# sebastianffx/stainlib

Hardware: AMD Instinct MI355X
Metric: 1024x1024 H&E tiles/sec normalized (Macenko) (higher is better)
Workload: dtype f32; 1 GPU; configs[1]: batch of 512 tiles 1024x1024x3 uint8 per GPU, Macenko transform (fit once outside the timed region), tiles resident in HBM; tiles_per_gpu=512, failed_tiles=0

## Files before the change

stainlib_amd/csrc/stats_finish.hpp:

```cpp
#pragma once
#include "stats_selection.hpp"
#include "stats_sweeps.hpp"

namespace sl {

struct SampleAngleKey {
    const uint32_t* sample; TabView tab; float V[6]; int cps_log2; int P; float ylimf;
    __device__ __forceinline__ float operator()(int b) const {
        if (sample_absent(b, cps_log2, P)) return nan_f();
        return of_word(sample[b]);
    }
    __device__ __forceinline__ float of_word(uint32_t s) const {
        const uint32_t r = s & 255u, g = (s >> 8) & 255u, bl = (s >> 16) & 255u;
        const bool tissue = is_tissue_f(tab.gam(r), tab.gam(g), tab.gam(bl), ylimf);
        const float k = angle_key(V, tab.odf(r), tab.odf(g), tab.odf(bl));
        return tissue ? k : nan_f();
    }
    __device__ __forceinline__ bool present(int b, int n_sample) const { return b < n_sample && !sample_absent(b, cps_log2, P); }
};
struct SampleConcKey {
    const uint32_t* sample; TabView tab; LassoK L; int cps_log2; int P; int col;
    __device__ __forceinline__ void both(int b, float& c1, float& c2) const {
        if (sample_absent(b, cps_log2, P)) { c1 = c2 = nan_f(); return; }
        of_word(sample[b], c1, c2);
    }
    __device__ __forceinline__ void of_word(uint32_t s, float& c1, float& c2) const {
        lasso2(L, tab.odf(s & 255u), tab.odf((s >> 8) & 255u), tab.odf((s >> 16) & 255u), c1, c2);
    }
    __device__ __forceinline__ bool present(int b, int n_sample) const { return b < n_sample && !sample_absent(b, cps_log2, P); }
    __device__ __forceinline__ float operator()(int b) const {
        float c1, c2;
        both(b, c1, c2);
        return col == 0 ? c1 : c2;
    }
};
struct AngleTileKey {
    const uint8_t* src; TabView tab; float V[6]; float ylimf;
    __device__ __forceinline__ float operator()(int p) const {
        const uint32_t r = src[3 * (size_t)p], g = src[3 * (size_t)p + 1], b = src[3 * (size_t)p + 2];
        if (!is_tissue_f(tab.gam(r), tab.gam(g), tab.gam(b), ylimf)) return nan_f();
        return angle_key(V, tab.odf(r), tab.odf(g), tab.odf(b));
    }
};
struct ConcTileKey {
    const uint8_t* src; TabView tab; LassoK L; int col;
    __device__ __forceinline__ float operator()(int p) const {
        float c1, c2;
        lasso2(L, tab.odf(src[3 * (size_t)p]), tab.odf(src[3 * (size_t)p + 1]), tab.odf(src[3 * (size_t)p + 2]), c1, c2);
        return col == 0 ? c1 : c2;
    }
};
struct RawConcKey2 {
    const uint32_t* raw; TabView tab; LassoK L;
    __device__ __forceinline__ void operator()(int i, float& k0, float& k1) const {
        const uint32_t s = raw[i];
        lasso2(L, tab.odf(s & 255u), tab.odf((s >> 8) & 255u), tab.odf((s >> 16) & 255u), k0, k1);
    }
};

struct CandKey {
    const float* cand;
    __device__ __forceinline__ float operator()(int i) const { return cand[i]; }
};

template <class Key2>
__device__ __forceinline__ void wg_refine(int n_raw, const Key2& key2, const float* lo, const float* hi, float* cand0,
                                          float* cand1, uint32_t cap_list, uint32_t* n_lt , uint32_t* n_in ,
                                          SelScratch& S, uint32_t* n_valid = nullptr ) {
    if (threadIdx.x < 4) S.misc[12 + threadIdx.x] = 0;
    if (threadIdx.x == 4) S.misc[8] = 0;
    __syncthreads();
    const int lane = threadIdx.x & 63;
    uint32_t lt0 = 0, lt1 = 0, nv = 0;
    constexpr int U = 4;
    const int step = (int)blockDim.x * U;
    for (int i0 = (int)(threadIdx.x - lane) * U; i0 < n_raw; i0 += step) {
        float k0[U], k1[U];
        unsigned long long m0[U], m1[U];
        uint32_t tot0 = 0, tot1 = 0;
#pragma unroll
        for (int u = 0; u < U; ++u) {
            const int i = i0 + u * 64 + lane;
            k0[u] = k1[u] = nan_f();
            if (i < n_raw) key2(i, k0[u], k1[u]);
        }
// ... 233 lines not shown
        if (__builtin_expect(n + cnt > stage_cap, 0)) flush(lane);
        const uint32_t rank = __builtin_amdgcn_mbcnt_hi((uint32_t)(m >> 32), __builtin_amdgcn_mbcnt_lo((uint32_t)m, 0u));
#if defined(__HIP_DEVICE_COMPILE__)
        uint32_t sbase;
        asm("s_lshl2_add_u32 %0, %1, %2" : "=s"(sbase) : "s"(n), "s"(buf) : "scc");
        const uint32_t addr = sbase + 4u * rank;
        unsigned long long saved;
        asm volatile("s_mov_b64 %0, exec\n\ts_mov_b64 exec, %1\n\tds_write_b32 %2, %3\n\ts_mov_b64 exec, %0"
                     : "=&s"(saved) : "s"(m), "v"(addr), "v"(value) : "memory");
#else
        (void)rank; (void)value;
#endif
        n += cnt;
    }
};


constexpr uint32_t kFinTabBytes = 2048;
__device__ __forceinline__ uint32_t fin_stage_bytes(int nthreads) { return (uint32_t)((sizeof(RowTab) - kFinTabBytes) / (size_t)(nthreads / 64)); }

struct FinTab {
    uint32_t base;
    __device__ __forceinline__ uint32_t addr(uint32_t w, int k) const { return k == 0 ? ((w << 3) & 0x7f8u) : ((w >> (8 * k - 3)) & 0x7f8u); }
#if defined(__HIP_DEVICE_COMPILE__)
    __device__ __forceinline__ float2 gam_odf(uint32_t a) const {
        const v2f v = *(SL_LDS const v2f*)(base + a);
        return make_float2(v.x, v.y);
    }
    __device__ __forceinline__ float odf(uint32_t a) const { return *(SL_LDS const float*)(base + a + 4u); }
#else
    float2 gam_odf(uint32_t) const { return float2{}; }
    float odf(uint32_t) const { return 0.0f; }
#endif
    __device__ __forceinline__ TabView view() const { return TabView{base, 8u, 4u, 0u}; }
};
__device__ __forceinline__ void fin_tab_build(RowTab& tab) {
    float2* p = reinterpret_cast<float2*>(tab.e);
    float2 e = make_float2(0.0f, 0.0f);
    if (threadIdx.x < 256) e = p[threadIdx.x * 32];
    __syncthreads();
    if (threadIdx.x < 256) p[threadIdx.x] = e;
    __syncthreads();
}

template <int NT>
__device__ __forceinline__ void fin_tab_expand(RowTab& tab) {
    float2* p = reinterpret_cast<float2*>(tab.e);
    constexpr int PER = 256 * 32 / NT;
    float2 e[PER];
#pragma unroll
    for (int j = 0; j < PER; ++j) e[j] = p[threadIdx.x / 32 + j * (NT / 32)];
    __syncthreads();
#pragma unroll
    for (int j = 0; j < PER; ++j) p[threadIdx.x + j * NT] = e[j];
    __syncthreads();
}

struct WordAngleKey {
    FinTab T; float V[6]; float ylimf;
    __device__ __forceinline__ void of_word(uint32_t s, float& k0, float& k1, bool& valid) const {
        const float2 er = T.gam_odf(T.addr(s, 0)), eg = T.gam_odf(T.addr(s, 1)), eb = T.gam_odf(T.addr(s, 2));
        valid = is_tissue_f(er.x, eg.x, eb.x, ylimf);
        k0 = k1 = angle_key(V, er.y, eg.y, eb.y);
    }
};
struct WordConcKey {
    FinTab T; LassoK L;
    __device__ __forceinline__ void of_word(uint32_t s, float& k0, float& k1, bool& valid) const {
        lasso2(L, T.odf(T.addr(s, 0)), T.odf(T.addr(s, 1)), T.odf(T.addr(s, 2)), k0, k1);
        valid = true;
    }
};

__device__ __forceinline__ void lds_count_masked(unsigned long long m, uint32_t addr, uint32_t one) {
#if defined(__HIP_DEVICE_COMPILE__)
    unsigned long long saved;
    asm volatile("s_mov_b64 %0, exec\n\ts_mov_b64 exec, %1\n\tds_add_u32 %2, %3\n\ts_mov_b64 exec, %0"
                 : "=&s"(saved) : "s"(m), "v"(addr), "v"(one) : "memory");
#else
    (void)m; (void)addr; (void)one;
#endif
}

struct RefineOut { uint32_t n_lt[2], n_in[2], n_valid; PickScale ps; };
template <class WordKey2>
__device__ __forceinline__ RefineOut wg_refine_s(const uint32_t* raw, int n_raw, const WordKey2& key2, float lo0, float hi0, float lo1, float hi1,
                                                 float* cand0, float* cand1, uint32_t cap_list, uint32_t stage_lds, uint32_t stage_entries,
                                                 SelScratch& S) {
    const int tid = threadIdx.x, lane = tid & 63;
    if (tid < 5) S.misc[8 + tid] = 0;
    for (int i = tid; i < 1024; i += blockDim.x) S.hist[i] = 0;
    RefineOut r;
    r.ps.lo[0] = lo0; r.ps.lo[1] = lo1;
    r.ps.sc[0] = (hi0 > lo0 && lo0 > -INFINITY && hi0 < INFINITY) ? 512.0f * 0.999999f / (hi0 - lo0) : 0.0f;
    r.ps.sc[1] = (hi1 > lo1 && lo1 > -INFINITY && hi1 < INFINITY) ? 512.0f * 0.999999f / (hi1 - lo1) : 0.0f;
    __syncthreads();
    stage_lds = (uint32_t)__builtin_amdgcn_readfirstlane((int)stage_lds);
    RawSink s0{stage_lds, 0u, reinterpret_cast<uint32_t*>(cand0), &S.misc[11], nullptr, cap_list, stage_entries};
    RawSink s1{stage_lds + 4u * stage_entries, 0u, reinterpret_cast<uint32_t*>(cand1), &S.misc[12], nullptr, cap_list, stage_entries};
    const float vlo0 = in_vgpr(lo0), vhi0 = in_vgpr(hi0), vlo1 = in_vgpr(lo1), vhi1 = in_vgpr(hi1);
    const float psl0 = in_vgpr(r.ps.lo[0]), psc0 = in_vgpr(r.ps.sc[0]), psl1 = in_vgpr(r.ps.lo[1]), psc1 = in_vgpr(r.ps.sc[1]);
    const uint32_t hist_lds = lds_address(S.hist);
    uint32_t one = 1u;
    asm("" : "+v"(one));
    uint32_t lt0 = 0, lt1 = 0, nv = 0;
    constexpr int U = 4;
    const int step = (int)blockDim.x * U;
    const int last = n_raw > 0 ? n_raw - 1 : 0;
    int i0 = (tid - lane) * U;
    uint32_t wn[U];
#pragma unroll
    for (int u = 0; u < U; ++u) wn[u] = as_global(raw)[min(i0 + u * 64 + lane, last)];
    for (; i0 < n_raw; i0 += step) {
        uint32_t w[U];
#pragma unroll
        for (int u = 0; u < U; ++u) {
            w[u] = wn[u];
            wn[u] = as_global(raw)[min(i0 + step + u * 64 + lane, last)];
        }
#pragma unroll
        for (int u = 0; u < U; ++u) {
            float k0, k1;
            bool valid;
            key2.of_word(w[u], k0, k1, valid);
            const bool inb = i0 + u * 64 + lane < n_raw;
            const unsigned long long mv = __builtin_amdgcn_ballot_w64(valid) & __builtin_amdgcn_ballot_w64(inb);
            const unsigned long long l0 = __builtin_amdgcn_ballot_w64(k0 < vlo0) & mv, l1 = __builtin_amdgcn_ballot_w64(k1 < vlo1) & mv;
            const unsigned long long m0 = __builtin_amdgcn_ballot_w64(k0 <= vhi0) & ~l0 & mv, m1 = __builtin_amdgcn_ballot_w64(k1 <= vhi1) & ~l1 & mv;
            nv += (uint32_t)__popcll(mv);
            lt0 += (uint32_t)__popcll(l0);
            lt1 += (uint32_t)__popcll(l1);
            lds_count_masked(m0, hist_lds + 4u * (uint32_t)pick_bin(k0, psl0, psc0), one);
            lds_count_masked(m1, hist_lds + 2048u + 4u * (uint32_t)pick_bin(k1, psl1, psc1), one);
            s0.put_value(m0, __float_as_uint(k0), lane);
            s1.put_value(m1, __float_as_uint(k1), lane);
        }
    }
    s0.flush(lane);
    s1.flush(lane);
    if (lane == 0) { if (nv) atomicAdd(&S.misc[8], nv); if (lt0) atomicAdd(&S.misc[9], lt0); if (lt1) atomicAdd(&S.misc[10], lt1); }
    __threadfence_block();
    __syncthreads();
    r.n_lt[0] = S.misc[9]; r.n_lt[1] = S.misc[10]; r.n_in[0] = S.misc[11]; r.n_in[1] = S.misc[12]; r.n_valid = S.misc[8];
    __syncthreads();
    return r;
}

constexpr float kBoxZ = 3.6f;
template <int THREADS>
__device__ __forceinline__ void angle_brackets(const SampleAngleKey& key, int n_sample, double pct, float* lo, float* hi,
                                               SelScratch& S, float* box = nullptr, float zs = 1.0f) {
    constexpr int KPT = kMaxSample / THREADS;
    uint32_t ord[1][KPT];
#ifdef SL_DEBUG_SUBCLK
    long long bclk_t_ = wall_clock64();
#endif
    static_assert(KPT % kBrkBatch == 0, "");
#pragma unroll
    for (int j0 = 0; j0 < KPT; j0 += kBrkBatch) {
        uint32_t w[kBrkBatch];
#pragma unroll
        for (int g = 0; g < kBrkBatch; ++g) {
            const int b = (j0 + g) * THREADS + (int)threadIdx.x;
            w[g] = b < n_sample ? as_global(key.sample)[b] : 0u;
        }
#pragma unroll
        for (int g = 0; g < kBrkBatch; ++g) {
            const int b = (j0 + g) * THREADS + (int)threadIdx.x;
            const float k = key.of_word(w[g]);
            ord[0][j0 + g] = (k == k && key.present(b, n_sample)) ? f2ord(k) : kAbsent;
        }
    }
    SL_BCLK(5);
    const int set_of[2] = {0, 0};
    const double p2[2] = {100.0 - pct, pct};
    wg_brackets_regs<1, KPT, 2>(ord, set_of, p2, lo, hi, S, kBracketZ * zs);
    if (box) {
        const bool closed = (lo[0] > -INFINITY) & (hi[0] < INFINITY) & (lo[1] > -INFINITY) & (hi[1] < INFINITY);
        if (closed) {
#pragma unroll
            for (int b = 0; b < 2; ++b) {
                const float m = 0.5f * (lo[b] + hi[b]), r = (float)kBoxFrac * 0.5f * (hi[b] - lo[b]);
                box[2 * b] = m - r; box[2 * b + 1] = m + r;
            }
        } else {
            const double n = (double)S.misc[6], q = p2[0] / 100.0;
            const bool inside = n > 0.0 && floor(q * (n - 1.0) - (double)(kBoxZ * zs) * sqrt(fmax(q * (1.0 - q) * n, 0.0))) - 1.0 >= 0.0;
            float blo[2] = {-INFINITY, -INFINITY}, bhi[2] = {INFINITY, INFINITY};
            __syncthreads();
            if (inside) wg_brackets_regs<1, KPT, 2>(ord, set_of, p2, blo, bhi, S, kBoxZ * zs);
            box[0] = blo[0]; box[1] = bhi[0]; box[2] = blo[1]; box[3] = bhi[1];
        }
    }
}
template <int THREADS>
__device__ __forceinline__ void conc_brackets(const SampleConcKey& key, int n_sample, float* lo, float* hi, SelScratch& S, float zs = 1.0f) {
    constexpr int KPT = kMaxSample / THREADS;
    uint32_t ord[2][KPT];
#ifdef SL_DEBUG_SUBCLK
    long long bclk_t_ = wall_clock64();
#endif
    static_assert(KPT % kBrkBatch == 0, "");
#pragma unroll
    for (int j0 = 0; j0 < KPT; j0 += kBrkBatch) {
        uint32_t w[kBrkBatch];
#pragma unroll
        for (int g = 0; g < kBrkBatch; ++g) {
            const int b = (j0 + g) * THREADS + (int)threadIdx.x;
            w[g] = b < n_sample ? as_global(key.sample)[b] : 0u;
        }
#pragma unroll
        for (int g = 0; g < kBrkBatch; ++g) {
            const int b = (j0 + g) * THREADS + (int)threadIdx.x;
            float c1, c2;
            key.of_word(w[g], c1, c2);
            const bool have = key.present(b, n_sample);
            ord[0][j0 + g] = (have && c1 == c1) ? f2ord(c1) : kAbsent;
            ord[1][j0 + g] = (have && c2 == c2) ? f2ord(c2) : kAbsent;
        }
    }
    SL_BCLK(6);
    const int set_of[2] = {0, 1};
    const double p2[2] = {99.0, 99.0};
    wg_brackets_regs<2, KPT, 2>(ord, set_of, p2, lo, hi, S, kBracketZ * zs);
}

}
```

stainlib_amd/csrc/stats_fused.hpp:

```cpp
#pragma once
#include "stats_phase_kernels.hpp"
#include "stats_cube.hpp"
#include "stats_twosweep.hpp"

namespace sl {

struct FusedArgs {
    const uint8_t* rgb;
    uint8_t* out;
    int n_tiles;
    int P;
    int stride_log2;
    int n_sample;
    float ylimf;
    double lam;
    double pct;
    const double* M_tgt;
    const double* maxC_tgt;
    int cap_raw, cap_list;
    uint32_t* raw;
    int cap_ang;
    uint32_t* raw_ang;
    float* cand;
    uint32_t* sample;
// ... 273 lines not shown
    const int P = __builtin_amdgcn_readfirstlane(P_), stream = __builtin_amdgcn_readfirstlane(stream_);
    const double lam = uni_d(lam_);
    const int tid = threadIdx.x;
    const TabReaderB TB = TabReaderB::make_at(FusedLds<NT>::tab);
    const int nch = (P + 3) >> 2;
    ApplyK K;
    apply_consts(sh.M, sh.maxC, M_tgt, maxC_tgt, lam, K);
    int t, c0, c1;
    fused_geometry<NT>(nch, tid, t, c0, c1);
    if (c0 >= c1) return;
    if (K.fast) {
        if (stream) apply_sweep<ALIGNED, true, TabReaderB, true>(src, dst, P, c0, c1, t, kFusedThreads, TB, K);
        else apply_sweep<ALIGNED, true, TabReaderB, false>(src, dst, P, c0, c1, t, kFusedThreads, TB, K);
    } else {
        if (stream) apply_sweep<ALIGNED, false, TabReaderB, true>(src, dst, P, c0, c1, t, kFusedThreads, TB, K);
        else apply_sweep<ALIGNED, false, TabReaderB, false>(src, dst, P, c0, c1, t, kFusedThreads, TB, K);
    }
}

template <int NT, bool ALIGNED>
__device__ __noinline__ void fused_sweep2_cube(FusedShared<NT>* shp, const uint8_t* src_, uint32_t* rawl_, uint32_t* rawa_, int P_, int cap_raw_, int cap_ang_,
                                               float ylimf_, int stream_) {
    FusedShared<NT>& sh = *shp;
    const uint8_t* src = uni_ptr(src_);
    uint32_t* rawl = uni_ptr(rawl_);
    uint32_t* rawa = uni_ptr(rawa_);
    const int P = __builtin_amdgcn_readfirstlane(P_), cap_raw = __builtin_amdgcn_readfirstlane(cap_raw_), stream = __builtin_amdgcn_readfirstlane(stream_);
    const int cap_ang = __builtin_amdgcn_readfirstlane(cap_ang_);
    const float ylimf = uni(ylimf_);
    const int tid = threadIdx.x, wave = tid >> 6;
    const TabReaderB TB = TabReaderB::make_at(FusedLds<NT>::tab);
    const int nch = (P + 3) >> 2;
    SelConsts K;
    for (int i = 0; i < 6; ++i) K.V[i] = in_vgpr(sh.Vf[i]);
    K.L.g12 = 0.0f;
    K.xmin = -INFINITY;
#pragma unroll
    for (int i = 0; i < 2; ++i) {
        K.u[i][0] = in_vgpr(sh.mk.u[i][0]); K.u[i][1] = in_vgpr(sh.mk.u[i][1]); K.kt[i] = in_vgpr(sh.mk.kt[i]);
        K.eps[i] = in_vgpr(sh.mk.eps[i]); K.thr[i] = in_vgpr(sh.mk.thr[i]);
    }
    K.lo0 = uni(sh.lo[0]); K.hi0 = uni(sh.hi[0]); K.lo1 = uni(sh.lo[1]); K.hi1 = uni(sh.hi[1]);
    static_assert(offsetof(FusedShared<NT>, n_ang) == offsetof(FusedShared<NT>, n_raw) + 4 && offsetof(FusedShared<NT>, n_raw) % 8 == 0, "");
    const RawDirect direct{rawl, rawa, reinterpret_cast<unsigned long long*>(&sh.n_raw), (uint32_t)cap_raw, (uint32_t)cap_ang};
    static_assert(offsetof(FusedShared<NT>, S) % 4096 == 0 && offsetof(SelScratch, hist) == 0, "the cube mask must be 4 KB aligned");
    const uint32_t bits_lds = FusedLds<NT>::hist;
    const uint32_t ring_lds = (uint32_t)__builtin_amdgcn_readfirstlane((int)(FusedLds<NT>::stage + (uint32_t)wave * FusedLds<NT>::stage_wave));
    int t, c0, c1;
    fused_geometry<NT>(nch, tid, t, c0, c1);
    if (c0 >= c1) return;
    if (stream) select_sweep_cube<ALIGNED, kFusedTrip, true>(src, P, c0, c1, t, kFusedThreads, TB, ylimf, K, bits_lds, ring_lds, direct);
    else select_sweep_cube<ALIGNED, kFusedTrip, false>(src, P, c0, c1, t, kFusedThreads, TB, ylimf, K, bits_lds, ring_lds, direct);
}

template <int NT>
__device__ SL_FINISH_ATTR int fused_finish2(FusedShared<NT>* shp, const uint8_t* src_, uint32_t* rawl_, uint32_t* rawa_, float* cand0_, float* cand1_, int P_,
                                          int cap_raw_, int cap_ang_, int cap_list_, float ylimf_, double pct_, double lam_, long long* subclk_, int ts_ = 0) {
    FusedShared<NT>& sh = *shp;
    const uint8_t* src = uni_ptr(src_);
    uint32_t* rawl = uni_ptr(rawl_);
    uint32_t* rawa = uni_ptr(rawa_);
    const int cap_ang = __builtin_amdgcn_readfirstlane(cap_ang_);
    float* cand0 = uni_ptr(cand0_);
    float* cand1 = uni_ptr(cand1_);
    const int P = __builtin_amdgcn_readfirstlane(P_), cap_raw = __builtin_amdgcn_readfirstlane(cap_raw_), cap_list = __builtin_amdgcn_readfirstlane(cap_list_);
    const float ylimf = uni(ylimf_);
    const double pct = uni_d(pct_), lam = uni_d(lam_);
    long long* subclk = uni_ptr(subclk_);
    const int ts = __builtin_amdgcn_readfirstlane(ts_);
    const int tid = threadIdx.x, wave = tid >> 6;
    int fallbacks = 0;
    (void)subclk;
    const uint32_t T = (uint32_t)sh.sum[0];
    long long k[2];
    {
        double g;
        percentile_pos((double)T, 100.0 - pct, k[0], g);
        percentile_pos((double)T, pct, k[1], g);
    }
    fin_tab_build(sh.tab);
    const FinTab FT{FusedLds<NT>::tab};
    const uint32_t stage_lds = FusedLds<NT>::tab + kFinTabBytes + (uint32_t)wave * fin_stage_bytes(NT);
    const uint32_t stage_entries = fin_stage_bytes(NT) / 8u;
    const auto tile_angle_key = [shp, src, ylimf](int) {
        AngleTileKey tkey;
        tkey.src = src; tkey.tab = FinTab{FusedLds<NT>::tab}.view(); tkey.ylimf = ylimf;
        for (int i = 0; i < 6; ++i) tkey.V[i] = shp->Vf[i];
        return tkey;
    };
    WordAngleKey rkey;
    rkey.T = FT; rkey.ylimf = ylimf;
    for (int i = 0; i < 6; ++i) rkey.V[i] = sh.Vf[i];
    const bool complete = sh.n_raw <= (uint32_t)cap_raw && sh.overflow == 0;
    const uint32_t n_raw = sh.n_raw < (uint32_t)cap_raw ? sh.n_raw : (uint32_t)cap_raw;
    const bool split = rawa != nullptr;
    const bool complete_a = split ? sh.n_ang <= (uint32_t)cap_ang : complete;
    const uint32_t n_a = split ? (sh.n_ang < (uint32_t)cap_ang ? sh.n_ang : (uint32_t)cap_ang) : n_raw;
    const uint32_t* lista = split ? rawa : rawl;
    const float los[2] = {sh.lo[0], sh.lo[1]}, his[2] = {sh.hi[0], sh.hi[1]};
    SL_SUB(2);
    const RefineOut ra = wg_refine_s(lista, (int)n_a, rkey, los[0], his[0], los[1], his[1], cand0, cand1, (uint32_t)cap_list, stage_lds,
                                     stage_entries, sh.S);
    SL_SUB(3);
    {
        const long long lt[2] = {(long long)ra.n_lt[0], (long long)T - (long long)ra.n_valid + (long long)ra.n_lt[1]};
        if (ts) {
            bool covered = complete_a;
#pragma unroll
            for (int b = 0; b < 2; ++b) {
                const long long k2 = (k[b] + 1 < (long long)T) ? k[b] + 1 : k[b];
                covered = covered & (k[b] >= lt[b]) & (k2 < lt[b] + (long long)ra.n_in[b]) & (ra.n_in[b] <= (uint32_t)cap_list);
            }
            if (!covered) {
                fin_tab_expand<NT>(sh.tab);
                return -1;
            }
        }
        float res[4];
        stage_pick2(cand0, cand1, ra.n_in, (uint32_t)cap_list, complete_a, los, his, lt, P, tile_angle_key, T, k, ra.ps, res, fallbacks, sh.S);
        if (tid == 0) { sh.res[0] = res[0]; sh.res[1] = res[1]; sh.res[2] = res[2]; sh.res[3] = res[3]; }
        __syncthreads();
    }
    SL_SUB(5);
    if (tid < 64) {
        double M[6];
        long long kd;
        double g0, g1;
        percentile_pos((double)T, 100.0 - pct, kd, g0);
        percentile_pos((double)T, pct, kd, g1);
        stain_matrix_from_angles(sh.Vd, sh.res, g0, g1, M, tid);
        if (tid == 0) {
            for (int i = 0; i < 6; ++i) sh.M[i] = M[i];
            if (stain_matrix_singular(M)) sh.status = SL_TILE_DEGENERATE_COV;
            const bool use = sh.status == SL_TILE_OK && complete && merged_verify(sh.mk, M, lam);
            sh.conc_done = use ? 1 : 0;
            sh.why = use ? 0 : (!sh.mk.ok ? SL_RESWEEP_NO_BOX : (!complete ? SL_RESWEEP_LIST_FULL : SL_RESWEEP_OUTSIDE_BOX));
            if (use) { LassoK L; lasso_consts(M, lam, L); sh.L = L; }
        }
    }
    __syncthreads();
    SL_SUB(6);
    if (sh.conc_done) {
        long long kc;
        double gc;
        percentile_pos((double)P, 99.0, kc, gc);
        const long long kc2 = kc + 1 < (long long)P ? kc + 1 : kc;
        WordConcKey ckey2;
        ckey2.T = FT; ckey2.L = sh.L;
        const float cl[2] = {sh.mk.L[0], sh.mk.L[1]}, chh[2] = {sh.mk.H[0], sh.mk.H[1]};
        const RefineOut rc = wg_refine_s(rawl, (int)n_raw, ckey2, cl[0], chh[0], cl[1], chh[1], cand0, cand1, (uint32_t)cap_list,
                                         stage_lds, stage_entries, sh.S);
        SL_SUB(14);
#ifdef SL_DEBUG_SUBCLK
        if (subclk && tid == 0) {
            long long* q = subclk;
            q[8] = 100ll * n_a; q[9] = 100ll * n_raw; q[10] = 100ll * (ra.n_in[0] + ra.n_in[1]); q[11] = 100ll * (rc.n_in[0] + rc.n_in[1]);
        }
#endif
        const long long n_plain = (long long)P - (long long)sh.n_raw;
        const long long clt[2] = {n_plain + rc.n_lt[0], n_plain + rc.n_lt[1]};
        bool covered = true;
#pragma unroll
        for (int col = 0; col < 2; ++col)
            covered = covered & (kc >= clt[col]) & (kc2 < clt[col] + (long long)rc.n_in[col]) & (rc.n_in[col] <= (uint32_t)cap_list);
        if (covered) {
            const auto tile_conc_key = [shp, src](int col) {
                ConcTileKey ctk;
                ctk.src = src; ctk.tab = FinTab{FusedLds<NT>::tab}.view(); ctk.L = shp->L; ctk.col = col;
                return ctk;
            };
            const long long kk[2] = {kc, kc};
            float res[4];
            stage_pick2(cand0, cand1, rc.n_in, (uint32_t)cap_list, true, cl, chh, clt, P, tile_conc_key, (uint32_t)P, kk, rc.ps, res, fallbacks, sh.S);
            if (tid == 0) {
                sh.maxC[0] = np_lerp((double)res[0], (double)res[1], gc);
                sh.maxC[1] = np_lerp((double)res[2], (double)res[3], gc);
                if (!(sh.maxC[0] > 0.0) || !(sh.maxC[1] > 0.0)) sh.status = SL_TILE_ZERO_MAXC;
            }
        } else if (tid == 0) {
            sh.conc_done = 0;
            sh.why = (rc.n_in[0] > (uint32_t)cap_list || rc.n_in[1] > (uint32_t)cap_list) ? SL_RESWEEP_LIST_FULL : SL_RESWEEP_BRACKET_MISSED;
        }
        __syncthreads();
        SL_SUB(15);
    }
    fin_tab_expand<NT>(sh.tab);
    return fallbacks;
}

template <int NT>
__device__ __noinline__ void phase0_estimate(FusedShared<NT>* shp, int mode_) {
    FusedShared<NT>& sh = *shp;
    const int mode = __builtin_amdgcn_readfirstlane(mode_);
    double Vd[6], wv[3];
    float Vf[6];
    const int st = eigvecs_from_moments(sh.sum, Vd, Vf, wv);
    const double ns = sh.sum[0];
    const double l1 = wv[0], l2 = wv[1], l3 = wv[2] > 0.0 ? wv[2] : 0.0;
    bool ok = st == SL_TILE_OK && ns >= (double)kTsMinTissue && l2 > 1e-9 * l1 && l2 - l3 > 0.05 * l2;
    double tau = 0.0;
    if (ok) {
        tau = kTiltZ * sqrt(kClusterDeff / ns) * fmax(sqrt(l3 * l2) / (l2 - l3), sqrt(l3 * l1) / (l1 - l3));
        tau = fmax(tau, kTsMinTau);
        ok = tau <= (mode >= 2 ? kTsMaxTau : kTsAutoMaxTau);
    }
    double nd[3] = {Vd[2] * Vd[5] - Vd[4] * Vd[3], Vd[4] * Vd[1] - Vd[0] * Vd[5], Vd[0] * Vd[3] - Vd[2] * Vd[1]};
    const double nn = 1.0 / sqrt(nd[0] * nd[0] + nd[1] * nd[1] + nd[2] * nd[2]);
    if (mode == 4 && ok) {
        double b[3];
        for (int c = 0; c < 3; ++c) b[c] = Vd[2 * c + 1] + 0.05 * nd[c] * nn;
        const double nb = 1.0 / sqrt(b[0] * b[0] + b[1] * b[1] + b[2] * b[2]);
        for (int c = 0; c < 3; ++c) { Vd[2 * c + 1] = b[c] * nb; Vf[2 * c + 1] = (float)Vd[2 * c + 1]; }
        nd[0] = Vd[2] * Vd[5] - Vd[4] * Vd[3]; nd[1] = Vd[4] * Vd[1] - Vd[0] * Vd[5]; nd[2] = Vd[0] * Vd[3] - Vd[2] * Vd[1];
    }
    const double nn2 = 1.0 / sqrt(nd[0] * nd[0] + nd[1] * nd[1] + nd[2] * nd[2]);
    for (int i = 0; i < 6; ++i) { sh.ts.Vd[i] = Vd[i]; sh.Vd[i] = Vd[i]; sh.Vf[i] = Vf[i]; }
    for (int c = 0; c < 3; ++c) { sh.ts.nd[c] = nd[c] * nn2; sh.ts.fn[c] = (float)(nd[c] * nn2); }
    sh.ts.tau = tau;
    sh.ts.gH[0] = l1 - l3; sh.ts.gH[1] = l2 - l3;
    sh.res[0] = (float)(4.0 * sqrt(l3));
    sh.res[1] = (float)(sh.sum[1] / ns); sh.res[2] = (float)(sh.sum[2] / ns); sh.res[3] = (float)(sh.sum[3] / ns);
    sh.status = ok ? SL_TILE_OK : SL_TILE_DEGENERATE_COV;
}

template <int NT>
__device__ __noinline__ void phase0_cone_and_box(FusedShared<NT>* shp, float hi0_, float lo1_, double lam_) {
    FusedShared<NT>& sh = *shp;
    const float hi0 = uni(hi0_), lo1 = uni(lo1_);
    const double lam = uni_d(lam_);
    const int tid = threadIdx.x;
    const double aH = angle_of_pseudo((double)hi0), aL = angle_of_pseudo((double)lo1);
    double sH, cH, sL, cL;
    sincos(aH, &sH, &cH);
    sincos(aL, &sL, &cL);
    if (tid == 0) {
        const double k2 = sh.ts.kappa2 + 6e-6;
        for (int c = 0; c < 3; ++c) {
            const double gH = sh.ts.Vd[2 * c] * -sH + sh.ts.Vd[2 * c + 1] * cH, gL = sh.ts.Vd[2 * c] * sL + sh.ts.Vd[2 * c + 1] * -cL;
            sh.ts.gH[c] = gH; sh.ts.gL[c] = gL;
            sh.ts.fgH[c] = (float)(gH - k2); sh.ts.fgL[c] = (float)(gL - k2);
        }
        sh.ts.fk1 = (float)(sh.ts.kappa1 * (1.0 + 1e-6));
        sh.ts.lo0 = sh.lo[0]; sh.ts.hi1 = sh.hi[1];
    }
    ts_box(sh.ts.Vd, sh.ts.nd, sh.ts.tau, sh.box, lam, tid, sh.mk);
}

template <int NT>
struct SampleRows {
    const uint32_t* samp;
    int n_sample, tid;
    uint32_t nx[kBrkBatch];
    __device__ __forceinline__ SampleRows(const uint32_t* s, int n, int t) : samp(s), n_sample(n), tid(t) {
        asm volatile("" : "+v"(tid));
        load(0);
    }
    __device__ __forceinline__ void load(int j0) {
#pragma unroll
        for (int u = 0; u < kBrkBatch; ++u) nx[u] = as_global(samp)[min((j0 + u) * NT + tid, n_sample - 1)];
    }
    __device__ __forceinline__ void next(uint32_t* w, int j0) {
#pragma unroll
        for (int u = 0; u < kBrkBatch; ++u) w[u] = nx[u];
        if (j0 + kBrkBatch < kMaxSample / NT) load(j0 + kBrkBatch);
    }
};

constexpr int kP0Bins = 1024;
// ... 698 lines not shown
```

Measured before the change: 386,500 tiles/s.

## Keep percentile candidates in LDS via sampled histogram window in refine

Adds a windowed variant of the refine sweep. A quick sample pass builds a histogram, picks a bin window sized to fit per-wave LDS staging, and writes only in-window candidates to LDS instead of spilling them to global candidate lists. A new LDS-based pick then finds the order statistics from these lists. When the window misses, overflows, or sampling is not allowed, the code falls back to a second full refine sweep plus the old global pick, which adds extra passes in those cases.

```diff
diff --git a/stainlib_amd/csrc/finish_window.hpp b/stainlib_amd/csrc/finish_window.hpp
--- /dev/null
+++ b/stainlib_amd/csrc/finish_window.hpp
@@ -0,0 +1,82 @@
+#pragma once
+#include <stdint.h>
+
+#if defined(__HIPCC__)
+#define SL_FINWIN_FN __host__ __device__ __forceinline__
+#else
+#define SL_FINWIN_FN inline
+#endif
+
+namespace sl {
+
+constexpr uint32_t kFinWinBins = 512;
+constexpr uint32_t kFinWinTrip = 256;
+constexpr uint32_t kFinWinSampleTrips = 2;
+constexpr uint32_t kFinWinFillNum = 3, kFinWinFillDen = 4;
+
+struct FinWindow { uint32_t lo, width; };
+struct FinRank { uint32_t beyond; int from_top; };
+
+SL_FINWIN_FN uint64_t fin_window_per_wave(uint32_t n_list, uint32_t nwaves) {
+    const uint64_t trip = (uint64_t)nwaves * kFinWinTrip;
+    return (((uint64_t)n_list + trip - 1) / trip) * kFinWinTrip;
+}
+
+SL_FINWIN_FN bool fin_window_all(uint32_t n_list, uint32_t nwaves, uint32_t cap_wave) {
+    return n_list > 0 && nwaves > 0 && fin_window_per_wave(n_list, nwaves) <= cap_wave;
+}
+
+SL_FINWIN_FN uint32_t fin_window_budget(uint32_t n_list, uint32_t n_sample, uint32_t nwaves, uint32_t cap_wave) {
+    if (n_list == 0 || n_sample == 0) return 0;
+    const uint64_t keys = (uint64_t)nwaves * cap_wave * kFinWinFillNum / kFinWinFillDen;
+    const uint64_t q = keys / n_list, rem = keys % n_list;
+    if (q > 0xffffffffull || q * n_sample > 0xffffffffull) return 0xffffffffu;
+    const uint64_t b = q * n_sample + rem * n_sample / n_list;
+    return b > 0xffffffffull ? 0xffffffffu : (uint32_t)b;
+}
+
+SL_FINWIN_FN int fin_window_centre(const uint32_t* cum, uint32_t n_out, FinRank r, uint32_t n_sample, uint32_t n_list) {
+    const uint32_t total = cum[kFinWinBins - 1];
+    const uint64_t rs = n_list ? (uint64_t)r.beyond * n_sample / n_list : 0;
+    if (rs < n_out) return r.from_top ? (int)kFinWinBins - 1 : 0;
+    const uint64_t want = rs - n_out;
+    if (want >= total) return r.from_top ? 0 : (int)kFinWinBins - 1;
+    int lo = 0, hi = (int)kFinWinBins - 1;
+    if (!r.from_top) {
+        while (lo < hi) { const int mid = (lo + hi) >> 1; if (cum[mid] > want) hi = mid; else lo = mid + 1; }
+        return lo;
+    }
+    while (lo < hi) {
+        const int mid = (lo + hi + 1) >> 1;
+        if ((uint64_t)total - cum[mid - 1] > want) lo = mid; else hi = mid - 1;
+    }
+    return lo;
+}
+
+SL_FINWIN_FN FinWindow fin_window_fit(const uint32_t* cum, int centre, uint32_t budget) {
+    const int c = centre < 0 ? 0 : (centre > (int)kFinWinBins - 1 ? (int)kFinWinBins - 1 : centre);
+    int lo = 0, hi = (int)kFinWinBins - 1;
+    while (lo < hi) {
+        const int h = (lo + hi + 1) >> 1;
+        const int a = c - h < 0 ? 0 : c - h, b = c + h > (int)kFinWinBins - 1 ? (int)kFinWinBins - 1 : c + h;
+        const uint32_t n = cum[b] - (a > 0 ? cum[a - 1] : 0u);
+        if (n <= budget) lo = h; else hi = h - 1;
+    }
+    const int a = c - lo < 0 ? 0 : c - lo, b = c + lo > (int)kFinWinBins - 1 ? (int)kFinWinBins - 1 : c + lo;
+    return FinWindow{(uint32_t)a, (uint32_t)(b - a + 1)};
+}
+
+SL_FINWIN_FN bool fin_window_hopeless(const uint32_t* cum, int centre, uint32_t budget, uint32_t n_sample, uint32_t n_list) {
+    const int c = centre < 0 ? 0 : (centre > (int)kFinWinBins - 1 ? (int)kFinWinBins - 1 : centre);
+    const uint32_t in_bin = cum[c] - (c > 0 ? cum[c - 1] : 0u);
+    return in_bin > budget || (uint64_t)in_bin * n_list >= 1024ull * (uint64_t)(n_sample ? n_sample : 1u);
+}
+
+SL_FINWIN_FN FinWindow fin_window_forced(FinWindow w) {
+#ifdef SL_FINWIN_FORCE_WIDTH
+    w.width = (uint32_t)(SL_FINWIN_FORCE_WIDTH) < w.width ? (uint32_t)(SL_FINWIN_FORCE_WIDTH) : w.width;
+#endif
+    return w;
+}
+
+}
diff --git a/stainlib_amd/csrc/stats_finish.hpp b/stainlib_amd/csrc/stats_finish.hpp
--- a/stainlib_amd/csrc/stats_finish.hpp
+++ b/stainlib_amd/csrc/stats_finish.hpp
@@ -1,6 +1,7 @@
 #pragma once
 #include "stats_selection.hpp"
 #include "stats_sweeps.hpp"
+#include "finish_window.hpp"
 
 namespace sl {
 
@@ -400,31 +401,140 @@
 #endif
 }
 
-struct RefineOut { uint32_t n_lt[2], n_in[2], n_valid; PickScale ps; };
-template <class WordKey2>
+struct WinSink {
+    uint32_t buf;
+    uint32_t n;
+    uint32_t cap;
+    uint32_t over;
+    __device__ __forceinline__ void put_value(unsigned long long m, uint32_t value) {
+        uint32_t cnt = (uint32_t)__popcll(m);
+        if (n + cnt > cap) { over = 1u; m = 0ull; cnt = 0u; }
+        const uint32_t rank = __builtin_amdgcn_mbcnt_hi((uint32_t)(m >> 32), __builtin_amdgcn_mbcnt_lo((uint32_t)m, 0u));
+#if defined(__HIP_DEVICE_COMPILE__)
+        uint32_t sbase;
+        asm("s_lshl2_add_u32 %0, %1, %2" : "=s"(sbase) : "s"(n), "s"(buf) : "scc");
+        const uint32_t addr = sbase + 4u * rank;
+        unsigned long long saved;
+        asm volatile("s_mov_b64 %0, exec\n\ts_mov_b64 exec, %1\n\tds_write_b32 %2, %3\n\ts_mov_b64 exec, %0"
+                     : "=&s"(saved) : "s"(m), "v"(addr), "v"(value) : "memory");
+#else
+        (void)rank; (void)value;
+#endif
+        n += cnt;
+    }
+};
+constexpr int kWinFill = 32;
+#ifdef SL_FINWIN_FORCE_CAP
+__device__ __forceinline__ uint32_t fin_win_cap(uint32_t entries) { return entries < (uint32_t)(SL_FINWIN_FORCE_CAP) ? entries : (uint32_t)(SL_FINWIN_FORCE_CAP); }
+#else
+__device__ __forceinline__ uint32_t fin_win_cap(uint32_t entries) { return entries; }
+#endif
+
+__device__ __forceinline__ void wave_cumulate_512(uint32_t* hist, int lane) {
+    uint32_t h[8], s = 0;
+#pragma unroll
+    for (int j = 0; j < 8; ++j) { h[j] = hist[lane * 8 + j]; s += h[j]; }
+    uint32_t acc = wave_inclusive_scan(s) - s;
+#pragma unroll
+    for (int j = 0; j < 8; ++j) { acc += h[j]; hist[lane * 8 + j] = acc; }
+}
+
+struct RefineOut { uint32_t n_lt[2], n_in[2], n_valid; PickScale ps; FinWindow win[2]; int skipped; };
+template <bool WIN, class WordKey2>
 __device__ __forceinline__ RefineOut wg_refine_s(const uint32_t* raw, int n_raw, const WordKey2& key2, float lo0, float hi0, float lo1, float hi1,
                                                  float* cand0, float* cand1, uint32_t cap_list, uint32_t stage_lds, uint32_t stage_entries,
-                                                 SelScratch& S) {
+                                                 SelScratch& S, FinRank want0 = FinRank{0u, 0}, FinRank want1 = FinRank{0u, 0}, bool may_sample = true) {
     const int tid = threadIdx.x, lane = tid & 63;
     if (tid < 5) S.misc[8 + tid] = 0;
+    if (WIN && tid < 3) S.misc[16 + tid] = 0;
     for (int i = tid; i < 1024; i += blockDim.x) S.hist[i] = 0;
     RefineOut r;
     r.ps.lo[0] = lo0; r.ps.lo[1] = lo1;
     r.ps.sc[0] = (hi0 > lo0 && lo0 > -INFINITY && hi0 < INFINITY) ? 512.0f * 0.999999f / (hi0 - lo0) : 0.0f;
     r.ps.sc[1] = (hi1 > lo1 && lo1 > -INFINITY && hi1 < INFINITY) ? 512.0f * 0.999999f / (hi1 - lo1) : 0.0f;
+    r.win[0] = r.win[1] = FinWindow{0u, 0u};
+    r.skipped = 0;
+    r.n_lt[0] = r.n_lt[1] = r.n_in[0] = r.n_in[1] = r.n_valid = 0u;
     __syncthreads();
     stage_lds = (uint32_t)__builtin_amdgcn_readfirstlane((int)stage_lds);
     RawSink s0{stage_lds, 0u, reinterpret_cast<uint32_t*>(cand0), &S.misc[11], nullptr, cap_list, stage_entries};
     RawSink s1{stage_lds + 4u * stage_entries, 0u, reinterpret_cast<uint32_t*>(cand1), &S.misc[12], nullptr, cap_list, stage_entries};
+    WinSink w0{stage_lds, 0u, fin_win_cap(stage_entries), 0u}, w1{stage_lds + 4u * stage_entries, 0u, fin_win_cap(stage_entries), 0u};
     const float vlo0 = in_vgpr(lo0), vhi0 = in_vgpr(hi0), vlo1 = in_vgpr(lo1), vhi1 = in_vgpr(hi1);
     const float psl0 = in_vgpr(r.ps.lo[0]), psc0 = in_vgpr(r.ps.sc[0]), psl1 = in_vgpr(r.ps.lo[1]), psc1 = in_vgpr(r.ps.sc[1]);
     const uint32_t hist_lds = lds_address(S.hist);
     uint32_t one = 1u;
     asm("" : "+v"(one));
-    uint32_t lt0 = 0, lt1 = 0, nv = 0;
+    const int last = n_raw > 0 ? n_raw - 1 : 0;
+    uint32_t wlo0 = 0, wn0 = 0, wlo1 = 0, wn1 = 0;
+    if constexpr (WIN) {
+        const uint32_t nwaves = blockDim.x >> 6, wave = (uint32_t)tid >> 6;
+        if (fin_window_all((uint32_t)n_raw, nwaves, stage_entries)) {
+            r.win[0] = r.win[1] = FinWindow{0u, kFinWinBins};
+        } else if (!may_sample || n_raw <= 0) {
+            r.skipped = 1;
+            return r;
+        } else {
+            uint32_t out0 = 0, out1 = 0, ns = 0;
+            constexpr uint32_t kRows = 4u * kFinWinSampleTrips;
+#pragma unroll
+            for (uint32_t t = 0; t < kFinWinSampleTrips; ++t) {
+                uint32_t ws[4];
+                int at[4];
+#pragma unroll
+                for (int u = 0; u < 4; ++u) {
+                    at[u] = (int)(((unsigned long long)(uint32_t)n_raw * (wave * kRows + t * 4u + (uint32_t)u)) / (nwaves * kRows)) + lane;
+                    ws[u] = as_global(raw)[min(at[u], last)];
+                }
+#pragma unroll
+                for (int u = 0; u < 4; ++u) {
+                    float k0, k1;
+                    bool valid;
+                    key2.of_word(ws[u], k0, k1, valid);
+                    const unsigned long long mi = __builtin_amdgcn_ballot_w64(at[u] < n_raw);
+                    const unsigned long long mv = __builtin_amdgcn_ballot_w64(valid) & mi;
+                    const unsigned long long m0 = __builtin_amdgcn_ballot_w64((k0 >= vlo0) & (k0 <= vhi0)) & mv;
+                    const unsigned long long m1 = __builtin_amdgcn_ballot_w64((k1 >= vlo1) & (k1 <= vhi1)) & mv;
+                    const unsigned long long o0 = __builtin_amdgcn_ballot_w64(want0.from_top ? k0 > vhi0 : k0 < vlo0) & mv;
+                    const unsigned long long o1 = __builtin_amdgcn_ballot_w64(want1.from_top ? k1 > vhi1 : k1 < vlo1) & mv;
+                    ns += (uint32_t)__popcll(mi); out0 += (uint32_t)__popcll(o0); out1 += (uint32_t)__popcll(o1);
+                    lds_count_masked(m0, hist_lds + 4u * (uint32_t)pick_bin(k0, psl0, psc0), one);
+                    lds_count_masked(m1, hist_lds + 2048u + 4u * (uint32_t)pick_bin(k1, psl1, psc1), one);
+                }
+            }
+            if (lane == 0) { if (out0) atomicAdd(&S.misc[16], out0); if (out1) atomicAdd(&S.misc[17], out1); if (ns) atomicAdd(&S.misc[18], ns); }
+            __threadfence_block();
+            __syncthreads();
+            if (wave < 2u) {
+                uint32_t* cum = S.hist + 512 * wave;
+                wave_cumulate_512(cum, lane);
+                __threadfence_block();
+                if (lane == 0) {
+                    const uint32_t n_s = S.misc[18];
+                    const FinRank want = wave ? want1 : want0;
+                    const int centre = fin_window_centre(cum, S.misc[16 + wave], want, n_s, (uint32_t)n_raw);
+                    const uint32_t budget = fin_window_budget((uint32_t)n_raw, n_s, nwaves, stage_entries);
+                    FinWindow w = fin_window_fit(cum, centre, budget);
+                    if (fin_window_hopeless(cum, centre, budget, n_s, (uint32_t)n_raw)) w.width = 0u;
+                    S.misc[20 + 2 * wave] = w.lo; S.misc[21 + 2 * wave] = w.width;
+                }
+            }
+            __syncthreads();
+            r.win[0] = FinWindow{S.misc[20], S.misc[21]};
+            r.win[1] = FinWindow{S.misc[22], S.misc[23]};
+            __syncthreads();
+            for (int i = tid; i < 1024; i += blockDim.x) S.hist[i] = 0;
+            __syncthreads();
+            if (r.win[0].width == 0u || r.win[1].width == 0u) { r.skipped = 1; return r; }
+        }
+        r.win[0] = fin_window_forced(r.win[0]); r.win[1] = fin_window_forced(r.win[1]);
+        wlo0 = r.win[0].lo; wn0 = r.win[0].width; wlo1 = r.win[1].lo; wn1 = r.win[1].width;
+        asm("" : "+v"(wlo0), "+v"(wn0), "+v"(wlo1), "+v"(wn1));
+    }
+    uint32_t lt0 = 0, lt1 = 0, nv = 0, in0 = 0, in1 = 0;
     constexpr int U = 4;
+    static_assert(U * 64 == (int)kFinWinTrip, "fin_window_all counts a wave's entries in trips of U x 64");
     const int step = (int)blockDim.x * U;
-    const int last = n_raw > 0 ? n_raw - 1 : 0;
     int i0 = (tid - lane) * U;
     uint32_t wn[U];
 #pragma unroll
@@ -448,20 +558,141 @@
             nv += (uint32_t)__popcll(mv);
             lt0 += (uint32_t)__popcll(l0);
             lt1 += (uint32_t)__popcll(l1);
-            lds_count_masked(m0, hist_lds + 4u * (uint32_t)pick_bin(k0, psl0, psc0), one);
-            lds_count_masked(m1, hist_lds + 2048u + 4u * (uint32_t)pick_bin(k1, psl1, psc1), one);
-            s0.put_value(m0, __float_as_uint(k0), lane);
-            s1.put_value(m1, __float_as_uint(k1), lane);
-        }
-    }
-    s0.flush(lane);
-    s1.flush(lane);
+            const uint32_t b0 = (uint32_t)pick_bin(k0, psl0, psc0), b1 = (uint32_t)pick_bin(k1, psl1, psc1);
+            lds_count_masked(m0, hist_lds + 4u * b0, one);
+            lds_count_masked(m1, hist_lds + 2048u + 4u * b1, one);
+            if constexpr (WIN) {
+                in0 += (uint32_t)__popcll(m0);
+                in1 += (uint32_t)__popcll(m1);
+                w0.put_value(m0 & __builtin_amdgcn_ballot_w64(b0 - wlo0 < wn0), __float_as_uint(k0));
+                w1.put_value(m1 & __builtin_amdgcn_ballot_w64(b1 - wlo1 < wn1), __float_as_uint(k1));
+            } else {
+                s0.put_value(m0, __float_as_uint(k0), lane);
+                s1.put_value(m1, __float_as_uint(k1), lane);
+            }
+        }
+    }
+    if constexpr (WIN) {
+        if (lane == 0) {
+            if (in0) atomicAdd(&S.misc[11], in0);
+            if (in1) atomicAdd(&S.misc[12], in1);
+            S.misc[kWinFill + 2 * (tid >> 6)] = w0.n | (w0.over << 31);
+            S.misc[kWinFill + 2 * (tid >> 6) + 1] = w1.n | (w1.over << 31);
+        }
+    } else {
+        s0.flush(lane);
+        s1.flush(lane);
+    }
     if (lane == 0) { if (nv) atomicAdd(&S.misc[8], nv); if (lt0) atomicAdd(&S.misc[9], lt0); if (lt1) atomicAdd(&S.misc[10], lt1); }
     __threadfence_block();
     __syncthreads();
     r.n_lt[0] = S.misc[9]; r.n_lt[1] = S.misc[10]; r.n_in[0] = S.misc[11]; r.n_in[1] = S.misc[12]; r.n_valid = S.misc[8];
     __syncthreads();
+    (void)in0; (void)in1; (void)s0; (void)s1; (void)w0; (void)w1; (void)wlo0; (void)wn0; (void)wlo1; (void)wn1;
     return r;
+}
+
+struct WinLists {
+    uint32_t base, wave_bytes, entries;
+#if defined(__HIP_DEVICE_COMPILE__)
+    __device__ __forceinline__ float key(int v, int b, int i) const { return *(SL_LDS const float*)(base + (uint32_t)v * wave_bytes + 4u * ((uint32_t)b * entries + (uint32_t)i)); }
+#else
+    float key(int, int, int) const { return 0.0f; }
+#endif
+};
+
+__device__ __forceinline__ void wg_pick2_w(const WinLists& wl, const FinWindow* win, const uint32_t* n_in, const uint32_t* krel, const PickScale& ps,
+                                           float* xa , float* xb , bool* done , int* why , SelScratch& S) {
+    const int tid = threadIdx.x, lane = tid & 63, wave = tid >> 6, nwaves = (int)(blockDim.x >> 6);
+#pragma unroll
+    for (int b = 0; b < 2; ++b)
+        if (wave == b) wave_locate(S.hist + 512 * b, 512, krel[b], &S.misc[16 + 3 * b], lane);
+    if (tid < 2) { S.misc[24 + tid] = 0; S.misc[26 + tid] = 0xffffffffu; }
+    __syncthreads();
+    uint32_t bin[2], below[2], cnt[2];
+#pragma unroll
+    for (int b = 0; b < 2; ++b) {
+        bin[b] = S.misc[16 + 3 * b]; below[b] = S.misc[17 + 3 * b]; cnt[b] = S.misc[18 + 3 * b];
+        uint32_t over = 0;
+        for (int v = 0; v < nwaves; ++v) over |= S.misc[kWinFill + 2 * v + b] >> 31;
+        why[b] = !(bin[b] - win[b].lo < win[b].width) ? 1 : (over ? 2 : (!(cnt[b] <= 512u && cnt[b] > 0u) ? 4 : 0));
+        done[b] = __builtin_amdgcn_readfirstlane(why[b]) == 0;
+    }
+    __syncthreads();
+    float* list = reinterpret_cast<float*>(S.hist);
+#pragma unroll
+    for (int b = 0; b < 2; ++b) {
+        if (!done[b]) continue;
+        uint32_t best = 0xffffffffu;
+        for (int v = 0; v < nwaves; ++v) {
+            const int n = (int)(S.misc[kWinFill + 2 * v + b] & 0x7fffffffu);
+            for (int i = tid; i < n; i += (int)blockDim.x) {
+                const float k = wl.key(v, b, i);
+                const int kb = pick_bin(k, ps.lo[b], ps.sc[b]);
+                if (kb == (int)bin[b]) { const uint32_t pos = atomicAdd(&S.misc[24 + b], 1u); if (pos < 512u) list[512 * b + pos] = k; }
+                else if (kb > (int)bin[b]) best = min(best, f2ord(k));
+            }
+        }
+        for (int o = 32; o > 0; o >>= 1) best = min(best, (uint32_t)__shfl_xor((int)best, o, 64));
+        if (lane == 0 && best != 0xffffffffu) atomicMin(&S.misc[26 + b], best);
+    }
+    __syncthreads();
+    if (tid < 4) S.misc[28 + tid] = 0;
+    __syncthreads();
+#pragma unroll
+    for (int b = 0; b < 2; ++b) {
+        if (!done[b]) continue;
+        const uint32_t m = cnt[b], ra = krel[b] - below[b];
+        if ((uint32_t)tid < m) {
+            const float me = list[512 * b + tid];
+            uint32_t r = 0;
+            for (uint32_t j = 0; j < m; ++j) {
+                const float o = list[512 * b + j];
+                r += (o < me || (o == me && j < (uint32_t)tid)) ? 1u : 0u;
+            }
+            if (r == ra) S.misc[28 + 2 * b] = __float_as_uint(me);
+            if (r == ra + 1) S.misc[29 + 2 * b] = __float_as_uint(me);
+        }
+    }
+    __syncthreads();
+#pragma unroll
+    for (int b = 0; b < 2; ++b) {
+        if (!done[b]) continue;
+        xa[b] = __uint_as_float(S.misc[28 + 2 * b]);
+        const bool same_bin = krel[b] - below[b] + 1 < cnt[b];
+        const uint32_t nx = S.misc[26 + b];
+        const bool behind = n_in[b] > below[b] + cnt[b];
+        if (!same_bin && behind && nx == 0xffffffffu) { why[b] = 3; done[b] = false; }
+        xb[b] = same_bin ? __uint_as_float(S.misc[29 + 2 * b]) : (nx != 0xffffffffu ? ord2f(nx) : xa[b]);
+    }
+    __syncthreads();
+}
+
+__device__ __forceinline__ bool stage_pick2_win(const WinLists& wl, const FinWindow* win, const uint32_t* n_in, uint32_t cap_list, bool complete,
+                                                const float* lo, const float* hi, const long long* lt, uint32_t n, const long long* k,
+                                                const PickScale& ps, float* res , int* why , SelScratch& S) {
+    bool fast[2], has2[2];
+    uint32_t krel[2];
+#pragma unroll
+    for (int b = 0; b < 2; ++b) {
+        const long long k2 = (k[b] + 1 < (long long)n) ? k[b] + 1 : k[b];
+        has2[b] = k2 != k[b];
+        const bool covered = complete && k[b] >= lt[b] && k2 < lt[b] + (long long)n_in[b];
+        fast[b] = covered && lo[b] < hi[b] && n_in[b] <= cap_list;
+        krel[b] = fast[b] ? (uint32_t)(k[b] - lt[b]) : 0u;
+        why[b] = 5;
+    }
+    if (!(fast[0] & fast[1])) return false;
+    float xa[2] = {0, 0}, xb[2] = {0, 0};
+    bool done[2] = {false, false};
+    wg_pick2_w(wl, win, n_in, krel, ps, xa, xb, done, why, S);
+    if (!(done[0] & done[1])) return false;
+#pragma unroll
+    for (int b = 0; b < 2; ++b) {
+        res[2 * b] = xa[b];
+        res[2 * b + 1] = has2[b] ? xb[b] : xa[b];
+    }
+    return true;
 }
 
 constexpr float kBoxZ = 3.6f;
diff --git a/stainlib_amd/csrc/stats_fused.hpp b/stainlib_amd/csrc/stats_fused.hpp
--- a/stainlib_amd/csrc/stats_fused.hpp
+++ b/stainlib_amd/csrc/stats_fused.hpp
@@ -379,6 +379,7 @@
     const FinTab FT{FusedLds<NT>::tab};
     const uint32_t stage_lds = FusedLds<NT>::tab + kFinTabBytes + (uint32_t)wave * fin_stage_bytes(NT);
     const uint32_t stage_entries = fin_stage_bytes(NT) / 8u;
+    const WinLists wlists{FusedLds<NT>::tab + kFinTabBytes, fin_stage_bytes(NT), stage_entries};
     const auto tile_angle_key = [shp, src, ylimf](int) {
         AngleTileKey tkey;
         tkey.src = src; tkey.tab = FinTab{FusedLds<NT>::tab}.view(); tkey.ylimf = ylimf;
@@ -396,9 +397,12 @@
     const uint32_t* lista = split ? rawa : rawl;
     const float los[2] = {sh.lo[0], sh.lo[1]}, his[2] = {sh.hi[0], sh.hi[1]};
     SL_SUB(2);
-    const RefineOut ra = wg_refine_s(lista, (int)n_a, rkey, los[0], his[0], los[1], his[1], cand0, cand1, (uint32_t)cap_list, stage_lds,
-                                     stage_entries, sh.S);
+    RefineOut ra = wg_refine_s<true>(lista, (int)n_a, rkey, los[0], his[0], los[1], his[1], cand0, cand1, (uint32_t)cap_list, stage_lds,
+                                     stage_entries, sh.S, FinRank{(uint32_t)k[0], 0}, FinRank{T - 1u - (uint32_t)k[1], 1}, ts != 0);
+    const bool lists_a = ra.skipped != 0;
+    if (lists_a) ra = wg_refine_s<false>(lista, (int)n_a, rkey, los[0], his[0], los[1], his[1], cand0, cand1, (uint32_t)cap_list, stage_lds, stage_entries, sh.S);
     SL_SUB(3);
+    int why_a[2] = {0, 0};
     {
         const long long lt[2] = {(long long)ra.n_lt[0], (long long)T - (long long)ra.n_valid + (long long)ra.n_lt[1]};
         if (ts) {
@@ -414,7 +418,14 @@
             }
         }
         float res[4];
-        stage_pick2(cand0, cand1, ra.n_in, (uint32_t)cap_list, complete_a, los, his, lt, P, tile_angle_key, T, k, ra.ps, res, fallbacks, sh.S);
+        if (lists_a) {
+            why_a[0] = why_a[1] = 6;
+            stage_pick2(cand0, cand1, ra.n_in, (uint32_t)cap_list, complete_a, los, his, lt, P, tile_angle_key, T, k, ra.ps, res, fallbacks, sh.S);
+        } else if (!stage_pick2_win(wlists, ra.win, ra.n_in, (uint32_t)cap_list, complete_a, los, his, lt, T, k, ra.ps, res, why_a, sh.S)) {
+            const RefineOut rb = wg_refine_s<false>(lista, (int)n_a, rkey, los[0], his[0], los[1], his[1], cand0, cand1, (uint32_t)cap_list, stage_lds,
+                                                    stage_entries, sh.S);
+            stage_pick2(cand0, cand1, rb.n_in, (uint32_t)cap_list, complete_a, los, his, lt, P, tile_angle_key, T, k, rb.ps, res, fallbacks, sh.S);
+        }
         if (tid == 0) { sh.res[0] = res[0]; sh.res[1] = res[1]; sh.res[2] = res[2]; sh.res[3] = res[3]; }
         __syncthreads();
     }
@@ -445,15 +456,13 @@
         WordConcKey ckey2;
         ckey2.T = FT; ckey2.L = sh.L;
         const float cl[2] = {sh.mk.L[0], sh.mk.L[1]}, chh[2] = {sh.mk.H[0], sh.mk.H[1]};
-        const RefineOut rc = wg_refine_s(rawl, (int)n_raw, ckey2, cl[0], chh[0], cl[1], chh[1], cand0, cand1, (uint32_t)cap_list,
-                                         stage_lds, stage_entries, sh.S);
+        const FinRank cwant{(uint32_t)((long long)P - 1 - kc), 1};
+        RefineOut rc = wg_refine_s<true>(rawl, (int)n_raw, ckey2, cl[0], chh[0], cl[1], chh[1], cand0, cand1, (uint32_t)cap_list,
+                                         stage_lds, stage_entries, sh.S, cwant, cwant, ts != 0);
+        const bool lists_c = rc.skipped != 0;
+        if (lists_c) rc = wg_refine_s<false>(rawl, (int)n_raw, ckey2, cl[0], chh[0], cl[1], chh[1], cand0, cand1, (uint32_t)cap_list, stage_lds, stage_entries, sh.S);
         SL_SUB(14);
-#ifdef SL_DEBUG_SUBCLK
-        if (subclk && tid == 0) {
-            long long* q = subclk;
-            q[8] = 100ll * n_a; q[9] = 100ll * n_raw; q[10] = 100ll * (ra.n_in[0] + ra.n_in[1]); q[11] = 100ll * (rc.n_in[0] + rc.n_in[1]);
-        }
-#endif
+        int why_c[2] = {0, 0};
         const long long n_plain = (long long)P - (long long)sh.n_raw;
         const long long clt[2] = {n_plain + rc.n_lt[0], n_plain + rc.n_lt[1]};
         bool covered = true;
@@ -468,7 +477,14 @@
             };
             const long long kk[2] = {kc, kc};
             float res[4];
-            stage_pick2(cand0, cand1, rc.n_in, (uint32_t)cap_list, true, cl, chh, clt, P, tile_conc_key, (uint32_t)P, kk, rc.ps, res, fallbacks, sh.S);
+            if (lists_c) {
+                why_c[0] = why_c[1] = 6;
+                stage_pick2(cand0, cand1, rc.n_in, (uint32_t)cap_list, true, cl, chh, clt, P, tile_conc_key, (uint32_t)P, kk, rc.ps, res, fallbacks, sh.S);
+            } else if (!stage_pick2_win(wlists, rc.win, rc.n_in, (uint32_t)cap_list, true, cl, chh, clt, (uint32_t)P, kk, rc.ps, res, why_c, sh.S)) {
+                const RefineOut rd = wg_refine_s<false>(rawl, (int)n_raw, ckey2, cl[0], chh[0], cl[1], chh[1], cand0, cand1, (uint32_t)cap_list,
+                                                        stage_lds, stage_entries, sh.S);
+                stage_pick2(cand0, cand1, rd.n_in, (uint32_t)cap_list, true, cl, chh, clt, P, tile_conc_key, (uint32_t)P, kk, rd.ps, res, fallbacks, sh.S);
+            }
             if (tid == 0) {
                 sh.maxC[0] = np_lerp((double)res[0], (double)res[1], gc);
                 sh.maxC[1] = np_lerp((double)res[2], (double)res[3], gc);
@@ -480,7 +496,16 @@
         }
         __syncthreads();
         SL_SUB(15);
-    }
+#ifdef SL_DEBUG_SUBCLK
+        if (subclk && tid == 0) {
+            long long* q = subclk;
+            q[8] = 100ll * n_a; q[9] = 100ll * n_raw;
+            q[10] = 100ll * (ra.n_in[0] + ra.n_in[1]) + why_a[0] + 8 * why_a[1];
+            q[11] = 100ll * (rc.n_in[0] + rc.n_in[1]) + why_c[0] + 8 * why_c[1];
+        }
+#endif
+    }
+    (void)why_a;
     fin_tab_expand<NT>(sh.tab);
     return fallbacks;
 }
```

Result: no change. 393,600 tiles/s, median of 6 (+1.8%).
